# VITA-Group/SinNeRF

Measured on AMD Instinct MI355X. Metric: rendered rays/sec (64+64 samples), lego 400x400, higher is better.
Workload: dtype f32; 1 GPU; nerf_synthetic/lego-shaped 400x400 frame (160000 rays/GPU), N_samples=64, N_importance=64, eval render (perturb=0, noise_std=0, white_back), random-init teacher weights; points_per_ray=192, parallelism=rays sharded x1, no collective

## Files before the change

include/sinnerf_hip.h:

```cpp
#ifndef SINNERF_HIP_H
#define SINNERF_HIP_H
#include <stdint.h>
#ifdef __cplusplus
extern "C" {
#endif

#define SN_ABI_VERSION 5

#define SN_DTYPE_F32 0
#define SN_DTYPE_BF16 1
#define SN_DTYPE_BF16_STATE 2
#define SN_DTYPE_BF16X3 3
#define SN_DTYPE_F16 4
#define SN_DTYPE_CLASSIC_HEADS 0x100
#define SN_DTYPE_COMPILER_SCHEDULED 0x200
#define SN_DTYPE_EMB_BF16 0x400

#define SN_E_BADARG (-1)
#define SN_E_TOOLARGE (-2)
#define SN_E_MISSING_RNG (-3)
#define SN_E_UNSUPPORTED (-4)
#define SN_E_BADSHAPE (-5)

#define SN_FLAG_BF16_COMPILER_SCHEDULED 2
// ... 49 lines not shown
int sn_composite_backward(const float* raw, const float* z_vals, const float* rays, const float* noise, float noise_std,
                          long n_rays, int n_samples, int white_back, const float* g_rgb, const float* g_depth,
                          const float* g_weights, float* g_raw, void* stream);

long sn_ray_grads_workspace_bytes(long n_rays, int n_samples);
int sn_ray_grads(const float* w1, const float* w5, const float* wdir, int dtype, const void* g_acts, long slot_rows,
                 const float* rays, const float* z_vals, long n_rays, int n_samples, void* workspace, float* g_rays,
                 void* stream);

int sn_composite_backward_rays(const float* raw, const float* z_vals, const float* rays, const float* noise, float noise_std,
                               long n_rays, int n_samples, int white_back, const float* g_rgb, const float* g_depth,
                               const float* g_weights, float* g_raw, float* g_rays, void* stream);

int sn_mlp_forward_embedded(const void* blob, int dtype, const float* x, long n_rows, int ld, int sigma_only,
                            int flags, float* out, void* stream);

int sn_composite_forward(const float* raw, int has_rgb, const float* z_vals, const float* rays, const float* noise,
                         float noise_std, long n_rays, int n_samples, int white_back, float* rgb, float* depth,
                         float* weights, void* stream);

int sn_sample_pdf(const float* z_vals, const float* weights, const float* u, long n_rays, int n_samples,
                  int n_importance, float* z_fine, float* z_merged, void* stream);

int sn_sample_pdf_bins(const float* bins, const float* weights, const float* u, long n_rays, int n_bins,
                       int n_importance, float eps, float* samples, void* stream);


int sn_generate_rays(const float* c2w, int H, int W, float focal, float near, float far, int x0, int y0, int stride_x,
                     int stride_y, int patch_w, int patch_h, float* rays, void* stream);

long sn_generate_rays_backward_workspace_bytes(void);
int sn_generate_rays_backward(const float* g_rays, int H, int W, float focal, int x0, int y0, int stride_x, int stride_y,
                              int patch_w, int patch_h, void* workspace, float* g_c2w, void* stream);

int sn_adam_step(float* params, const float* grads, float* exp_avg, float* exp_avg_sq, long n, float lr, float beta1,
                 float beta2, float eps, float weight_decay, int step, void* stream);

long sn_render_loss_workspace_bytes(void);
int sn_render_loss(const float* rgb_coarse, const float* rgb_fine, const float* depth_coarse, const float* depth_fine,
                   const float* rgb_gt, const float* depth_gt, const unsigned char* mask, int mask_mode, long n,
                   float w_rgb, float w_depth, float* g_rgb_coarse, float* g_rgb_fine, float* g_depth_coarse,
                   float* g_depth_fine, void* workspace, float* out, void* stream);

#ifdef __cplusplus
}
#endif
// ... 2 lines not shown
```

sinnerf_amd/_lib.py:

```python
import ctypes
import os

_HERE = os.path.dirname(os.path.abspath(__file__))
LIB_PATH = os.environ.get("SINNERF_HIP_LIB") or os.path.join(_HERE, "csrc", "libsinnerf_hip.so")

SN_DTYPE_F32 = 0
SN_DTYPE_BF16 = 1
SN_DTYPE_BF16_STATE = 2
SN_DTYPE_BF16X3 = 3
SN_DTYPE_F16 = 4
SN_DTYPE_CLASSIC_HEADS = 0x100
SN_FLAG_F32_LDS_RING = 4
SN_DTYPE_COMPILER_SCHEDULED = 0x200
N_RAW_TENSORS = 24
SN_DTYPE_EMB_BF16 = 0x400
ABI_VERSION = 5

c_fp = ctypes.c_void_p
c_vp = ctypes.c_void_p
_long, _int, _float = ctypes.c_long, ctypes.c_int, ctypes.c_float

SIGNATURES = {
    "sn_abi_version": (_int, []),
    "sn_error_string": (ctypes.c_char_p, [_int]),
# ... 18 lines not shown
    "sn_sample_coarse": (_int, [c_fp, _long, _int, _int, _float, c_fp, c_fp, c_vp]),
    "sn_mlp_forward": (_int, [c_vp, _int, c_fp, c_fp, _long, _int, _int, _int, c_fp, c_vp]),
    "sn_mlp_forward_train": (_int, [c_vp, _int, c_fp, c_fp, _long, _int, c_fp, c_fp, c_fp, _long, c_vp]),
    "sn_mlp_forward_train_embedded": (_int, [c_vp, _int, c_fp, _long, _int, c_fp, c_fp, _long, c_vp]),
    "sn_mlp_backward_chain": (_int, [c_vp, _int, c_fp, c_fp, c_fp, _long, _long, c_fp, c_fp, c_vp]),
    "sn_dw_gemm": (_int, [c_vp, _int, c_vp]),
    "sn_weight_grads_workspace_bytes": (_long, [_long, _int]),
    "sn_weight_grads_plan": (_int, [_long, _int, c_vp, _int]),
    "sn_weight_grads": (_int, [c_vp, c_fp, c_vp, _long, _int, c_vp, ctypes.POINTER(c_vp), _int, c_vp]),
    "sn_generate_rays": (_int, [c_fp, _int, _int, _float, _float, _float, _int, _int, _int, _int, _int, _int, c_fp, c_vp]),
    "sn_adam_step": (_int, [c_fp, c_fp, c_fp, c_fp, _long, _float, _float, _float, _float, _float, _int, c_vp]),
    "sn_render_loss_workspace_bytes": (_long, []),
    "sn_render_loss": (_int, [c_fp, c_fp, c_fp, c_fp, c_fp, c_fp, c_vp, _int, _long, _float, _float, c_fp, c_fp, c_fp, c_fp,
                              c_vp, c_fp, c_vp]),
    "sn_composite_backward": (_int, [c_fp, c_fp, c_fp, c_fp, _float, _long, _int, _int, c_fp, c_fp, c_fp, c_fp, c_vp]),
    "sn_ray_grads_workspace_bytes": (_long, [_long, _int]),
    "sn_ray_grads": (_int, [c_fp, c_fp, c_fp, _int, c_vp, _long, c_fp, c_fp, _long, _int, c_vp, c_fp, c_vp]),
    "sn_composite_backward_rays": (_int, [c_fp, c_fp, c_fp, c_fp, _float, _long, _int, _int, c_fp, c_fp, c_fp, c_fp, c_fp, c_vp]),
    "sn_generate_rays_backward_workspace_bytes": (_long, []),
    "sn_generate_rays_backward": (_int, [c_fp, _int, _int, _float, _int, _int, _int, _int, _int, _int, c_vp, c_fp, c_vp]),
    "sn_mlp_forward_embedded": (_int, [c_vp, _int, c_fp, _long, _int, _int, _int, c_fp, c_vp]),
    "sn_composite_forward": (_int, [c_fp, _int, c_fp, c_fp, c_fp, _float, _long, _int, _int, c_fp, c_fp, c_fp, c_vp]),
    "sn_sample_pdf": (_int, [c_fp, c_fp, c_fp, _long, _int, _int, c_fp, c_fp, c_vp]),
    "sn_sample_pdf_bins": (_int, [c_fp, c_fp, c_fp, _long, _int, _int, _float, c_fp, c_vp]),
}


class SinnerfHipError(RuntimeError):
    pass


def _load():
    if not os.path.exists(LIB_PATH):
        raise ImportError(
            f"{LIB_PATH} not found: the HIP extension is not built. Run `python -c 'import __graft_entry__ as g; "
            "g.build()'` (or `make -C sinnerf_amd/csrc`). There is no CPU fallback for this path.")
    lib = ctypes.CDLL(LIB_PATH)
    for name, (res, args) in SIGNATURES.items():
        fn = getattr(lib, name)
        fn.restype, fn.argtypes = res, args
    if lib.sn_abi_version() != ABI_VERSION:
        raise ImportError(f"{LIB_PATH}: ABI version {lib.sn_abi_version()} != {ABI_VERSION}; rebuild the extension")
    return lib


lib = _load()
# ... 19 lines not shown
```

sinnerf_amd/csrc/sn_api.hip:

```cpp
#include <hip/hip_fp16.h>
#include "../../include/sinnerf_hip.h"
#include "sn_device.h"
#include "sn_layout.h"

extern "C" {
int sn_mlp_forward_f32_launch(const void* blob, const float* in0, const float* in1, long n_points, int s_or_ld,
                              int sigma_only, int input_mode, float* out, float* acts, float* emb,
                              long slot_rows, hipStream_t stream);
int sn_mlp_forward_f32g_launch(const void* blob, const float* in0, const float* in1, long n_points, int s_or_ld, int sigma_only,
                               int input_mode, float* out, float* acts, float* emb, long slot_rows, hipStream_t stream);
int sn_mlp_forward_f32g_classic_launch(const void* blob, const float* in0, const float* in1, long n_points, int s_or_ld, int sigma_only,
                                       int input_mode, float* out, float* acts, float* emb, long slot_rows, hipStream_t stream);
int sn_mlp_forward_f32g_store_launch(const void* blob, const float* in0, const float* in1, long n_points, int s_or_ld, int sigma_only,
                                     int input_mode, float* out, float* acts, float* emb, long slot_rows, hipStream_t stream);
int sn_mlp_forward_f32g_store_classic_launch(const void* blob, const float* in0, const float* in1, long n_points, int s_or_ld, int sigma_only,
                                             int input_mode, float* out, float* acts, float* emb, long slot_rows, hipStream_t stream);
int sn_mlp_forward_f32_classic_launch(const void* blob, const float* in0, const float* in1, long n_points, int s_or_ld,
                              int sigma_only, int input_mode, float* out, float* acts, float* emb,
                              long slot_rows, hipStream_t stream);
int sn_mlp_backward_chain_f32_launch(const void* bblob, const float* acts, const float* out_raw, const float* g_raw,
                                     long n_points, long slot_rows, float* G, float* g_out, hipStream_t stream);
int sn_mlp_backward_chain_f32_classic_launch(const void* bblob, const float* acts, const float* out_raw, const float* g_raw,
                                     long n_points, long slot_rows, float* G, float* g_out, hipStream_t stream);
int sn_mlp_backward_chain_f32g_launch(const void* bblob, const float* acts, const float* out_raw, const float* g_raw, long n_points,
// ... 67 lines not shown
                                                long n_points, long slot_rows, float* G, float* g_out, hipStream_t stream);
int sn_composite_backward_launch(const float* raw, const float* z_vals, const float* rays, const float* noise,
                                 float noise_std, long n_rays, int n_samples, int white_back, const float* g_rgb,
                                 const float* g_depth, const float* g_w, float* g_raw, hipStream_t stream);
int sn_composite_backward_rays_launch(const float* raw, const float* z_vals, const float* rays, const float* noise,
                                      float noise_std, long n_rays, int n_samples, int white_back, const float* g_rgb,
                                      const float* g_depth, const float* g_w, float* g_raw, float* g_rays, hipStream_t stream);
long sn_ray_grads_workspace_bytes_impl(long n_rays, int n_samples);
int sn_ray_grads_launch(const float* w1, const float* w5, const float* wdir, int layout, const void* g_acts, long slot_rows,
                        const float* rays, const float* z_vals, long n_rays, int n_samples, void* workspace, float* g_rays,
                        hipStream_t stream);
long sn_generate_rays_backward_workspace_bytes_impl();
int sn_generate_rays_backward_launch(const float* g_rays, int H, int W, float focal, int x0, int y0, int sx, int sy, int pw,
                                     int ph, void* workspace, float* g_c2w, hipStream_t stream);
int sn_sample_coarse_launch(const float* rays, long n_rays, int n_samples, int use_disp, float perturb,
                            const float* perturb_rand, float* z_out, hipStream_t stream);
int sn_composite_forward_launch(const float* raw, int has_rgb, const float* z_vals, const float* rays,
                                const float* noise, float noise_std, long n_rays, int n_samples, int white_back,
                                float* rgb, float* depth, float* weights, hipStream_t stream);
int sn_sample_pdf_launch(const float* z_vals, const float* weights, const float* u, long n_rays, int n_samples,
                         int n_importance, float* z_fine, float* z_merged, hipStream_t stream);
int sn_sample_pdf_bins_launch(const float* bins, const float* weights, const float* u, long n_rays, int n_bins,
                              int n_importance, float eps, float* samples, hipStream_t stream);
}

namespace {
struct RawPtrs { const float* p[snl::N_RAW]; };

__device__ __forceinline__ unsigned short f32_to_bf16_rne(float f) {
  unsigned int u = __float_as_uint(f);
  if ((u & 0x7fffffffu) > 0x7f800000u) return (unsigned short)((u >> 16) | 0x40);
  u += 0x7fffu + ((u >> 16) & 1u);
  return (unsigned short)(u >> 16);
}

__global__ void __launch_bounds__(256)
pack_kernel(RawPtrs raw, const snl::PackEntry* __restrict__ table, long n, char* __restrict__ blob, int dtype) {
  for (long i = (long)blockIdx.x * blockDim.x + threadIdx.x; i < n; i += (long)gridDim.x * blockDim.x) {
    const snl::PackEntry e = table[i];
    float v = 0.0f;
    const bool as_f32 = (e.src == -2) || (e.src >= 0 && (e.src & snl::SRC_F32_FLAG));
    if (e.src >= 0) {
      const int t = (e.src >> 20) & 0x1ff, off = e.src & 0xfffff;
      const float* src = raw.p[0];
#pragma unroll
      for (int k = 1; k < snl::N_RAW; ++k) src = (t == k) ? raw.p[k] : src;
// ... 323 lines not shown
    return SN_HEADS(classic, sn_mlp_forward_bf16)(blob, x, nullptr, n_rows, ld, sigma_only, 1, out, nullptr, nullptr, 0, 0, (hipStream_t)stream);
  if (dtype != SN_DTYPE_F32) return SN_E_UNSUPPORTED;
  if (!(flags & SN_FLAG_F32_LDS_RING))
    return SN_HEADS(classic, sn_mlp_forward_f32g)(blob, x, nullptr, n_rows, ld, sigma_only, 1, out, nullptr, nullptr, 0, (hipStream_t)stream);
  return SN_HEADS(classic, sn_mlp_forward_f32)(blob, x, nullptr, n_rows, ld, sigma_only, 1,
                                               out, nullptr, nullptr, 0, (hipStream_t)stream);
}

int sn_composite_forward(const float* raw, int has_rgb, const float* z_vals, const float* rays, const float* noise,
                         float noise_std, long n_rays, int n_samples, int white_back, float* rgb, float* depth,
                         float* weights, void* stream) {
  if (!raw || !z_vals || !rays || !weights || n_rays < 0 || n_samples < 1) return SN_E_BADARG;
  if (has_rgb && (!rgb || !depth)) return SN_E_BADARG;
  return sn_composite_forward_launch(raw, has_rgb, z_vals, rays, noise, noise_std, n_rays, n_samples, white_back, rgb,
                                     depth, weights, (hipStream_t)stream);
}

int sn_sample_pdf(const float* z_vals, const float* weights, const float* u, long n_rays, int n_samples,
                  int n_importance, float* z_fine, float* z_merged, void* stream) {
  if (!z_vals || !weights || !z_merged || n_rays < 0) return SN_E_BADARG;
  return sn_sample_pdf_launch(z_vals, weights, u, n_rays, n_samples, n_importance, z_fine, z_merged, (hipStream_t)stream);
}

int sn_sample_pdf_bins(const float* bins, const float* weights, const float* u, long n_rays, int n_bins,
                       int n_importance, float eps, float* samples, void* stream) {
  if (!bins || !weights || !samples || n_rays < 0 || !(eps > 0.0f)) return SN_E_BADARG;
  return sn_sample_pdf_bins_launch(bins, weights, u, n_rays, n_bins, n_importance, eps, samples, (hipStream_t)stream);
}

}
```

sinnerf_amd/csrc/sn_render.hip:

```cpp
#include "sn_device.h"

namespace snr {

SN_DEV float linspace01(int i, int n) {
  if (n <= 1) return 0.0f;
  const float step = __fdiv_rn(1.0f, (float)(n - 1));
  return (i < n / 2) ? __fmul_rn((float)i, step) : __builtin_fmaf(-(float)(n - 1 - i), step, 1.0f);
}

SN_DEV float coarse_z(float near, float far, float t, int use_disp) {
  const float omt = __fsub_rn(1.0f, t);
  if (!use_disp) return __fadd_rn(__fmul_rn(near, omt), __fmul_rn(far, t));
  const float a = __fmul_rn(__fdiv_rn(1.0f, near), omt), b = __fmul_rn(__fdiv_rn(1.0f, far), t);
  return __fdiv_rn(1.0f, __fadd_rn(a, b));
}

__global__ void __launch_bounds__(256)
sample_coarse_kernel(const float* __restrict__ rays, long n_rays, int S, int use_disp, float perturb,
                     const float* __restrict__ perturb_rand, float* __restrict__ z_out) {
  const long total = n_rays * (long)S;
  for (long idx = (long)blockIdx.x * blockDim.x + threadIdx.x; idx < total; idx += (long)gridDim.x * blockDim.x) {
    const long ray = idx / S;
    const int i = (int)(idx - ray * S);
    const float near = rays[ray * 8 + 6], far = rays[ray * 8 + 7];
// ... 19 lines not shown
  return v;
}
SN_DEV double wave_incl_scan_add(double v, int lane) {
#pragma unroll
  for (int off = 1; off < 64; off <<= 1) {
    const double o = __shfl_up(v, off, 64);
    if (lane >= off) v += o;
  }
  return v;
}
SN_DEV double wave_sum(double v) {
#pragma unroll
  for (int off = 32; off > 0; off >>= 1) v += __shfl_xor(v, off, 64);
  return v;
}

SN_DEV void wave_lds_sync() {
  __builtin_amdgcn_fence(__ATOMIC_RELEASE, "wavefront");
  __builtin_amdgcn_wave_barrier();
  __builtin_amdgcn_fence(__ATOMIC_ACQUIRE, "wavefront");
}

template <int C, bool HAS_RGB>
__global__ void __launch_bounds__(256)
composite_fwd_kernel(const float* __restrict__ raw, const float* __restrict__ z_vals, const float* __restrict__ rays,
                     const float* __restrict__ noise, float noise_std, long n_rays, int S, int white_back,
                     float* __restrict__ rgb_out, float* __restrict__ depth_out, float* __restrict__ w_out) {
  const int lane = threadIdx.x & 63;
  const long ray = (long)blockIdx.x * 4 + (threadIdx.x >> 6);
  if (ray >= n_rays) return;
  const float dx = rays[ray * 8 + 3], dy = rays[ray * 8 + 4], dz = rays[ray * 8 + 5];
  const float dnorm = __fsqrt_rn(__fadd_rn(__fadd_rn(__fmul_rn(dx, dx), __fmul_rn(dy, dy)), __fmul_rn(dz, dz)));
  const long base = ray * (long)S;
  const int i0 = lane * C;

  float z[C + 1], sg[C], cr[C], cg[C], cb[C];
#pragma unroll
  for (int c = 0; c < C + 1; ++c) {
    const int i = i0 + c;
    z[c] = (i < S) ? z_vals[base + i] : 0.0f;
  }
#pragma unroll
  for (int c = 0; c < C; ++c) {
    const int i = i0 + c;
    if (i < S) {
      if (HAS_RGB) {
        const float4 v = reinterpret_cast<const float4*>(raw)[base + i];
        cr[c] = v.x; cg[c] = v.y; cb[c] = v.z; sg[c] = v.w;
      } else {
        sg[c] = raw[base + i];
        cr[c] = cg[c] = cb[c] = 0.0f;
      }
    } else {
      sg[c] = cr[c] = cg[c] = cb[c] = 0.0f;
    }
  }
  float alpha[C];
  double fprod = 1.0;
#pragma unroll
  for (int c = 0; c < C; ++c) {
    const int i = i0 + c;
    float a = 0.0f, f = 1.0f;
    if (i < S) {
      float delta = (i < S - 1) ? __fsub_rn(z[c + 1], z[c]) : 1e10f;
      delta = __fmul_rn(delta, dnorm);
      float s = sg[c];
      if (noise != nullptr) s = __fadd_rn(s, __fmul_rn(noise[base + i], noise_std));
      s = fmaxf(s, 0.0f);
      a = __fsub_rn(1.0f, expf(__fmul_rn(-delta, s)));
      f = __fadd_rn(__fsub_rn(1.0f, a), 1e-10f);
    }
    alpha[c] = a;
    fprod *= (double)f;
  }
  const double incl = wave_incl_scan_mul(fprod, lane);
  double t = __shfl_up(incl, 1, 64);
  if (lane == 0) t = 1.0;
  double wsum = 0.0, sr = 0.0, sgc = 0.0, sb = 0.0, sd = 0.0;
#pragma unroll
  for (int c = 0; c < C; ++c) {
    const int i = i0 + c;
    const float w = __fmul_rn(alpha[c], (float)t);
    if (i < S) {
      w_out[base + i] = w;
      wsum += (double)w;
      if (HAS_RGB) {
        sr += (double)__fmul_rn(w, cr[c]);
        sgc += (double)__fmul_rn(w, cg[c]);
        sb += (double)__fmul_rn(w, cb[c]);
        sd += (double)__fmul_rn(w, z[c]);
      }
      const float a = alpha[c];
      t *= (double)__fadd_rn(__fsub_rn(1.0f, a), 1e-10f);
    }
  }
  if (HAS_RGB) {
    wsum = wave_sum(wsum); sr = wave_sum(sr); sgc = wave_sum(sgc); sb = wave_sum(sb); sd = wave_sum(sd);
    if (lane == 0) {
      float r = (float)sr, g = (float)sgc, b = (float)sb;
      if (white_back) {
        const float ws = (float)wsum;
        r = __fsub_rn(__fadd_rn(r, 1.0f), ws);
        g = __fsub_rn(__fadd_rn(g, 1.0f), ws);
        b = __fsub_rn(__fadd_rn(b, 1.0f), ws);
      }
      rgb_out[ray * 3 + 0] = r; rgb_out[ray * 3 + 1] = g; rgb_out[ray * 3 + 2] = b;
      depth_out[ray] = (float)sd;
    }
  }
}

template <int C, bool RAYS>
SN_DEV void composite_bwd_body(const float* __restrict__ raw, const float* __restrict__ z_vals, const float* __restrict__ rays,
                               const float* __restrict__ noise, float noise_std, long n_rays, int S, int white_back,
                               const float* __restrict__ g_rgb, const float* __restrict__ g_depth,
                               const float* __restrict__ g_w, float* __restrict__ g_raw, float* __restrict__ g_rays) {
  const int lane = threadIdx.x & 63;
  const long ray = (long)blockIdx.x * 4 + (threadIdx.x >> 6);
  if (ray >= n_rays) return;
  const float dx = rays[ray * 8 + 3], dy = rays[ray * 8 + 4], dz = rays[ray * 8 + 5];
  const float dnorm = __fsqrt_rn(__fadd_rn(__fadd_rn(__fmul_rn(dx, dx), __fmul_rn(dy, dy)), __fmul_rn(dz, dz)));
  const long base = ray * (long)S;
  const int i0 = lane * C;
  const float gr = g_rgb ? g_rgb[ray * 3 + 0] : 0.0f, gg = g_rgb ? g_rgb[ray * 3 + 1] : 0.0f,
              gb = g_rgb ? g_rgb[ray * 3 + 2] : 0.0f, gd = g_depth ? g_depth[ray] : 0.0f;
  const float gwhite = white_back ? (gr + gg + gb) : 0.0f;

  float zc[C + 1];
#pragma unroll
  for (int c = 0; c < C + 1; ++c) zc[c] = (i0 + c < S) ? z_vals[base + i0 + c] : 0.0f;
  float alpha[C], ex[C], dl[C], Gi[C], fi[C];
  float dzs[C], sps[C];
// ... 62 lines not shown
      reinterpret_cast<float4*>(g_rays)[ray * 2] = lo;
      reinterpret_cast<float4*>(g_rays)[ray * 2 + 1] = hi;
    }
  }
}

template <int C>
__global__ void __launch_bounds__(256)
composite_bwd_kernel(const float* __restrict__ raw, const float* __restrict__ z_vals, const float* __restrict__ rays,
                     const float* __restrict__ noise, float noise_std, long n_rays, int S, int white_back,
                     const float* __restrict__ g_rgb, const float* __restrict__ g_depth, const float* __restrict__ g_w,
                     float* __restrict__ g_raw) {
  composite_bwd_body<C, false>(raw, z_vals, rays, noise, noise_std, n_rays, S, white_back, g_rgb, g_depth, g_w, g_raw, nullptr);
}
template <int C>
__global__ void __launch_bounds__(256)
composite_bwd_rays_kernel(const float* __restrict__ raw, const float* __restrict__ z_vals, const float* __restrict__ rays,
                          const float* __restrict__ noise, float noise_std, long n_rays, int S, int white_back,
                          const float* __restrict__ g_rgb, const float* __restrict__ g_depth, const float* __restrict__ g_w,
                          float* __restrict__ g_raw, float* __restrict__ g_rays) {
  composite_bwd_body<C, true>(raw, z_vals, rays, noise, noise_std, n_rays, S, white_back, g_rgb, g_depth, g_w, g_raw, g_rays);
}

template <bool FROM_Z>
__global__ void __launch_bounds__(256)
sample_pdf_kernel(const float* __restrict__ z_vals, const float* __restrict__ weights, const float* __restrict__ u_in,
                  long n_rays, int S, int NI, float eps, float* __restrict__ z_fine_out, float* __restrict__ z_merged_out) {
  extern __shared__ __attribute__((aligned(16))) char smem[];
  const int lane = threadIdx.x & 63;
  const int wv = threadIdx.x >> 6;
  const long ray = (long)blockIdx.x * 4 + wv;
  const int M = S - 2;
  const int L = S - 1;
  const int n = S + NI;
  const int per_wave = 2 * L + n + (FROM_Z ? n : 0);
  float* cdf = reinterpret_cast<float*>(smem) + (long)wv * per_wave;
  float* bins = cdf + L;
  float* keys = bins + L;
  float* merged = keys + n;
  if (ray >= n_rays) return;
  const long base = FROM_Z ? ray * (long)S : ray * (long)M - 1;

  const int C = (M + 63) / 64;
  double local = 0.0;
  for (int c = 0; c < C; ++c) {
    const int k = lane * C + c;
    if (k < M) local += (double)__fadd_rn(weights[base + k + 1], eps);
  }
  const float tot = (float)wave_sum(local);
  double run = 0.0;
  for (int c = 0; c < C; ++c) {
    const int k = lane * C + c;
    if (k < M) run += (double)__fdiv_rn(__fadd_rn(weights[base + k + 1], eps), tot);
  }
  const double incl = wave_incl_scan_add(run, lane);
  double acc = incl - run;
  for (int c = 0; c < C; ++c) {
    const int k = lane * C + c;
    if (k < M) {
      acc += (double)__fdiv_rn(__fadd_rn(weights[base + k + 1], eps), tot);
      cdf[k + 1] = (float)acc;
    }
  }
  if (lane == 0) cdf[0] = 0.0f;
  if (FROM_Z) {
    for (int k = lane; k < L; k += 64)
      bins[k] = __fmul_rn(0.5f, __fadd_rn(z_vals[base + k], z_vals[base + k + 1]));
    for (int k = lane; k < S; k += 64) keys[k] = z_vals[base + k];
  } else {
    for (int k = lane; k < L; k += 64) bins[k] = z_vals[ray * (long)L + k];
  }
  wave_lds_sync();

  for (int i = lane; i < NI; i += 64) {
    const float u = (u_in != nullptr) ? u_in[ray * (long)NI + i] : linspace01(i, NI);
    int lo = 0, hi = L;
    while (lo < hi) {
      const int mid = (lo + hi) >> 1;
      if (cdf[mid] <= u) lo = mid + 1; else hi = mid;
    }
    const int inds = lo;
    const int below = max(inds - 1, 0);
    const int above = min(inds, M);
    const float c0 = cdf[below], c1 = cdf[above], b0 = bins[below], b1 = bins[above];
    float denom = __fsub_rn(c1, c0);
    if (denom < eps) denom = 1.0f;
    const float smp = __fadd_rn(b0, __fmul_rn(__fdiv_rn(__fsub_rn(u, c0), denom), __fsub_rn(b1, b0)));
    keys[S + i] = smp;
    if (z_fine_out != nullptr) z_fine_out[ray * (long)NI + i] = smp;
  }
  if (!FROM_Z) return;
  wave_lds_sync();
  bool ascending = true;
  for (int i = lane; i < NI - 1; i += 64) ascending = ascending && (keys[S + i] <= keys[S + i + 1]);
  for (int i = lane; i < S - 1; i += 64) ascending = ascending && (keys[i] <= keys[i + 1]);
  if (__all(ascending)) {
    const float* kf = keys + S;
    for (int i = lane; i < S; i += 64) {
      const float k = keys[i];
      int lo = 0, hi = NI;
      while (lo < hi) {
        const int mid = (lo + hi) >> 1;
        if (kf[mid] < k) lo = mid + 1; else hi = mid;
      }
      merged[i + lo] = k;
    }
    for (int m = lane; m < NI; m += 64) {
      const float k = kf[m];
      int lo = 0, hi = S;
      while (lo < hi) {
        const int mid = (lo + hi) >> 1;
        if (keys[mid] <= k) lo = mid + 1; else hi = mid;
      }
      merged[m + lo] = k;
    }
  } else {
    for (int i = lane; i < n; i += 64) {
      const float k = keys[i];
      int rank = 0;
      for (int j = 0; j < n; ++j) {
        const float kj = keys[j];
        rank += (kj < k || (kj == k && j < i)) ? 1 : 0;
      }
      merged[rank] = k;
    }
  }
  wave_lds_sync();
  for (int i = lane; i < n; i += 64) z_merged_out[ray * (long)n + i] = merged[i];
}

}

extern "C" int sn_sample_coarse_launch(const float* rays, long n_rays, int n_samples, int use_disp, float perturb,
                                       const float* perturb_rand, float* z_out, hipStream_t stream) {
  if (n_rays <= 0) return 0;
  if (perturb > 0.0f && perturb_rand == nullptr) return -3;
  const long total = n_rays * (long)n_samples;
  long blocks = (total + 255) / 256;
  if (blocks > 256 * 16) blocks = 256 * 16;
  hipLaunchKernelGGL(snr::sample_coarse_kernel, dim3((unsigned)blocks), dim3(256), 0, stream, rays, n_rays, n_samples,
                     use_disp, perturb, perturb_rand, z_out);
  return (int)hipGetLastError();
}

extern "C" int sn_composite_forward_launch(const float* raw, int has_rgb, const float* z_vals, const float* rays,
                                           const float* noise, float noise_std, long n_rays, int n_samples,
                                           int white_back, float* rgb, float* depth, float* weights,
                                           hipStream_t stream) {
  using namespace snr;
  if (n_rays <= 0) return 0;
  const int C = (n_samples + 63) / 64;
// ... 52 lines not shown
    hipLaunchKernelGGL((composite_bwd_rays_kernel<CC>), grid, block, 0, stream, raw, z_vals, rays, noise, noise_std, n_rays, \
                       n_samples, white_back, g_rgb, g_depth, g_w, g_raw, g_rays);                               \
    break;
  switch (C) { SN_CBR(1) SN_CBR(2) SN_CBR(3) SN_CBR(4) SN_CBR(5) SN_CBR(6) SN_CBR(7) SN_CBR(8) SN_CBR(9) SN_CBR(10) SN_CBR(11)
               SN_CBR(12) SN_CBR(13) SN_CBR(14) SN_CBR(15) SN_CBR(16) }
#undef SN_CBR
  return (int)hipGetLastError();
}

extern "C" int sn_sample_pdf_launch(const float* z_vals, const float* weights, const float* u, long n_rays,
                                    int n_samples, int n_importance, float* z_fine, float* z_merged,
                                    hipStream_t stream) {
  if (n_rays <= 0) return 0;
  if (n_samples < 3 || n_importance < 1) return -5;
  const long blocks = (n_rays + 3) / 4;
  if (blocks > 0x7fffffffL) return -2;
  const size_t lds = 4 * (size_t)(2 * (n_samples - 1) + 2 * (n_samples + n_importance)) * sizeof(float);
  if (lds > 64 * 1024) return -4;
  hipLaunchKernelGGL(snr::sample_pdf_kernel<true>, dim3((unsigned)blocks), dim3(256), lds, stream, z_vals, weights, u,
                     n_rays, n_samples, n_importance, 1e-5f , z_fine, z_merged);
  return (int)hipGetLastError();
}

extern "C" int sn_sample_pdf_bins_launch(const float* bins, const float* weights, const float* u, long n_rays,
                                         int n_bins, int n_importance, float eps, float* samples, hipStream_t stream) {
  if (n_rays <= 0) return 0;
  if (n_bins < 1 || n_importance < 1) return -5;
  const int S = n_bins + 2;
  const long blocks = (n_rays + 3) / 4;
  if (blocks > 0x7fffffffL) return -2;
  const size_t lds = 4 * (size_t)(2 * (S - 1) + S + n_importance) * sizeof(float);
  if (lds > 64 * 1024) return -4;
  hipLaunchKernelGGL(snr::sample_pdf_kernel<false>, dim3((unsigned)blocks), dim3(256), lds, stream, bins, weights, u,
                     n_rays, S, n_importance, eps, samples, (float*)nullptr);
  return (int)hipGetLastError();
}
```

sinnerf_amd/rendering.py:

```python
import torch

from . import _lib
from .nerf import NeRF, dtype_code

__all__ = ["render_rays", "sample_pdf"]

PROFILE = None


MAX_FUSED_SAMPLES = 1024


def _is_pow2_bands(e, in_channels, n_freqs):
    fb = getattr(e, "freq_bands", None)
    if isinstance(fb, torch.Tensor):
        key = (id(fb), fb._version, fb.data_ptr(), tuple(fb.shape), str(fb.device), in_channels, n_freqs)
        if fb.device.type == "cpu" and fb.numel() <= 16:
            key += (tuple(fb.detach().reshape(-1).tolist()),)
    else:
        try:
            key = (tuple(float(v) for v in fb), in_channels, n_freqs) if fb is not None else (None, in_channels, n_freqs)
        except TypeError:
            key = (id(fb), in_channels, n_freqs)
    hit = getattr(e, "_sn_pow2_verdict", None)
    if hit is not None and hit[0] == key:
        return hit[1]
    ok = (fb is not None and getattr(e, "in_channels", None) == in_channels and getattr(e, "N_freqs", None) == n_freqs
          and len(fb) == n_freqs)
    if ok:
        host = torch.as_tensor(fb).detach().to("cpu", torch.float64)
        ok = bool(torch.equal(host, 2.0 ** torch.arange(n_freqs, dtype=torch.float64)))
# ... 57 lines not shown
        res.update(rgb_coarse=e(0, 3), depth_coarse=e(0))
    elif N_importance == 0:
        raise NameError("name 'rgb_coarse' is not defined (rendering.py:331)")
    res.update(rgb_fine=e(0, 3), depth_fine=e(0), opacity_fine=e(0, sf))
    return res


def _forward_core(models, rays, N_samples, use_disp, perturb, noise_std, N_importance, white_back, test_time,
                  flags=0, keep=None):
    dev = rays.device
    n = rays.shape[0]
    if n == 0:
        return _empty_result(dev, N_samples, N_importance, test_time)
    stream = _lib.stream_ptr()
    perturb_rand = None
    if perturb > 0:
        perturb_rand = torch.rand((n, N_samples), device=dev)
    z_vals = torch.empty((n, N_samples), dtype=torch.float32, device=dev)
    _lib.check(_lib.lib.sn_sample_coarse(_lib.ptr(rays), n, N_samples, int(bool(use_disp)), float(perturb),
                                         _lib.ptr(perturb_rand), _lib.ptr(z_vals), stream), "sn_sample_coarse")
    result = {}
    raw_c = _mlp(models[0], rays, z_vals, sigma_only=bool(test_time), flags=flags)
    noise_c = torch.randn((n, N_samples), device=dev)
    rgb_c, depth_c, w_c = _composite(raw_c, not test_time, z_vals, rays, noise_c if noise_std != 0 else None,
                                     noise_std, white_back)
    if test_time:
        result["opacity_coarse"] = w_c
    else:
        result.update(rgb_coarse=rgb_c, depth_coarse=depth_c, opacity_coarse=w_c)
    if keep is not None:
        keep.update(z_coarse=z_vals, raw_coarse=raw_c, noise_coarse=noise_c if noise_std != 0 else None)
    if N_importance > 0:
        u = torch.rand((n, N_importance), device=dev) if perturb > 0 else None
        z_all = torch.empty((n, N_samples + N_importance), dtype=torch.float32, device=dev)
        _lib.check(_lib.lib.sn_sample_pdf(_lib.ptr(z_vals), _lib.ptr(w_c), _lib.ptr(u), n, N_samples, N_importance,
                                          None, _lib.ptr(z_all), stream), "sn_sample_pdf")
        raw_f = _mlp(models[1], rays, z_all, sigma_only=False, flags=flags)
        noise_f = torch.randn((n, N_samples + N_importance), device=dev)
        rgb_f, depth_f, w_f = _composite(raw_f, True, z_all, rays, noise_f if noise_std != 0 else None, noise_std,
                                         white_back)
        result.update(rgb_fine=rgb_f, depth_fine=depth_f, opacity_fine=w_f)
        if keep is not None:
            keep.update(z_fine=z_all, raw_fine=raw_f, noise_fine=noise_f if noise_std != 0 else None)
    else:
        if test_time:
            raise NameError("name 'rgb_coarse' is not defined (render_rays(test_time=True) needs N_importance > 0, "
                            "as in the reference: rendering.py:331)")
        result.update(rgb_fine=rgb_c, depth_fine=depth_c, opacity_fine=w_c)
    return result


def render_rays(models,
                embeddings,
                rays,
                N_samples=64,
                use_disp=False,
                perturb=0,
                noise_std=1,
                N_importance=0,
# ... 59 lines not shown
```

Before: 661,600 rays/s.

## Fuse coarse compositing with PDF importance sampling into one persistent kernel

```diff
diff --git a/include/sinnerf_hip.h b/include/sinnerf_hip.h
--- a/include/sinnerf_hip.h
+++ b/include/sinnerf_hip.h
@@ -95,6 +95,10 @@
 int sn_sample_pdf(const float* z_vals, const float* weights, const float* u, long n_rays, int n_samples,
                   int n_importance, float* z_fine, float* z_merged, void* stream);
 
+int sn_coarse_tail(const float* raw, int has_rgb, const float* z_vals, const float* rays, const float* noise, float noise_std,
+                   const float* u, long n_rays, int n_samples, int n_importance, int white_back, float* rgb, float* depth,
+                   float* weights, float* z_all, void* stream);
+
 int sn_sample_pdf_bins(const float* bins, const float* weights, const float* u, long n_rays, int n_bins,
                        int n_importance, float eps, float* samples, void* stream);
 
diff --git a/sinnerf_amd/_lib.py b/sinnerf_amd/_lib.py
--- a/sinnerf_amd/_lib.py
+++ b/sinnerf_amd/_lib.py
@@ -64,6 +64,7 @@
     "sn_mlp_forward_embedded": (_int, [c_vp, _int, c_fp, _long, _int, _int, _int, c_fp, c_vp]),
     "sn_composite_forward": (_int, [c_fp, _int, c_fp, c_fp, c_fp, _float, _long, _int, _int, c_fp, c_fp, c_fp, c_vp]),
     "sn_sample_pdf": (_int, [c_fp, c_fp, c_fp, _long, _int, _int, c_fp, c_fp, c_vp]),
+    "sn_coarse_tail": (_int, [c_fp, _int, c_fp, c_fp, c_fp, _float, c_fp, _long, _int, _int, _int, c_fp, c_fp, c_fp, c_fp, c_vp]),
     "sn_sample_pdf_bins": (_int, [c_fp, c_fp, c_fp, _long, _int, _int, _float, c_fp, c_vp]),
 }
 
diff --git a/sinnerf_amd/csrc/sn_api.hip b/sinnerf_amd/csrc/sn_api.hip
--- a/sinnerf_amd/csrc/sn_api.hip
+++ b/sinnerf_amd/csrc/sn_api.hip
@@ -113,6 +113,9 @@
                          int n_importance, float* z_fine, float* z_merged, hipStream_t stream);
 int sn_sample_pdf_bins_launch(const float* bins, const float* weights, const float* u, long n_rays, int n_bins,
                               int n_importance, float eps, float* samples, hipStream_t stream);
+int sn_coarse_tail_launch(const float* raw, int has_rgb, const float* z_vals, const float* rays, const float* noise,
+                          float noise_std, const float* u, long n_rays, int n_samples, int n_importance, int white_back,
+                          float* rgb, float* depth, float* weights, float* z_all, hipStream_t stream);
 }
 
 namespace {
@@ -482,6 +485,15 @@
   return sn_sample_pdf_launch(z_vals, weights, u, n_rays, n_samples, n_importance, z_fine, z_merged, (hipStream_t)stream);
 }
 
+int sn_coarse_tail(const float* raw, int has_rgb, const float* z_vals, const float* rays, const float* noise, float noise_std,
+                   const float* u, long n_rays, int n_samples, int n_importance, int white_back, float* rgb, float* depth,
+                   float* weights, float* z_all, void* stream) {
+  if (!raw || !z_vals || !rays || !weights || !z_all || n_rays < 0 || n_samples < 1) return SN_E_BADARG;
+  if (has_rgb && (!rgb || !depth)) return SN_E_BADARG;
+  return sn_coarse_tail_launch(raw, has_rgb, z_vals, rays, noise, noise_std, u, n_rays, n_samples, n_importance, white_back,
+                               rgb, depth, weights, z_all, (hipStream_t)stream);
+}
+
 int sn_sample_pdf_bins(const float* bins, const float* weights, const float* u, long n_rays, int n_bins,
                        int n_importance, float eps, float* samples, void* stream) {
   if (!bins || !weights || !samples || n_rays < 0 || !(eps > 0.0f)) return SN_E_BADARG;
diff --git a/sinnerf_amd/csrc/sn_render.hip b/sinnerf_amd/csrc/sn_render.hip
--- a/sinnerf_amd/csrc/sn_render.hip
+++ b/sinnerf_amd/csrc/sn_render.hip
@@ -1,4 +1,5 @@
 #include "sn_device.h"
+#include "sn_launch.h"
 
 namespace snr {
 
@@ -65,39 +66,40 @@
 }
 
 template <int C, bool HAS_RGB>
-__global__ void __launch_bounds__(256)
-composite_fwd_kernel(const float* __restrict__ raw, const float* __restrict__ z_vals, const float* __restrict__ rays,
-                     const float* __restrict__ noise, float noise_std, long n_rays, int S, int white_back,
-                     float* __restrict__ rgb_out, float* __restrict__ depth_out, float* __restrict__ w_out) {
-  const int lane = threadIdx.x & 63;
-  const long ray = (long)blockIdx.x * 4 + (threadIdx.x >> 6);
-  if (ray >= n_rays) return;
-  const float dx = rays[ray * 8 + 3], dy = rays[ray * 8 + 4], dz = rays[ray * 8 + 5];
-  const float dnorm = __fsqrt_rn(__fadd_rn(__fadd_rn(__fmul_rn(dx, dx), __fmul_rn(dy, dy)), __fmul_rn(dz, dz)));
+struct CompIn {
+  float z[C + 1], sg[C], nz[C];
+  float cr[HAS_RGB ? C : 1], cg[HAS_RGB ? C : 1], cb[HAS_RGB ? C : 1];
+  float dx, dy, dz;
+};
+
+template <int C, bool HAS_RGB>
+SN_DEV void comp_load(CompIn<C, HAS_RGB>& in, const float* __restrict__ raw, const float* __restrict__ z_vals,
+                      const float* __restrict__ rays, const float* __restrict__ noise, long ray, int S, int lane) {
+  in.dx = rays[ray * 8 + 3]; in.dy = rays[ray * 8 + 4]; in.dz = rays[ray * 8 + 5];
   const long base = ray * (long)S;
   const int i0 = lane * C;
-
-  float z[C + 1], sg[C], cr[C], cg[C], cb[C];
-#pragma unroll
-  for (int c = 0; c < C + 1; ++c) {
-    const int i = i0 + c;
-    z[c] = (i < S) ? z_vals[base + i] : 0.0f;
-  }
+#pragma unroll
+  for (int c = 0; c < C + 1; ++c) in.z[c] = z_vals[base + min(i0 + c, S - 1)];
 #pragma unroll
   for (int c = 0; c < C; ++c) {
-    const int i = i0 + c;
-    if (i < S) {
-      if (HAS_RGB) {
-        const float4 v = reinterpret_cast<const float4*>(raw)[base + i];
-        cr[c] = v.x; cg[c] = v.y; cb[c] = v.z; sg[c] = v.w;
-      } else {
-        sg[c] = raw[base + i];
-        cr[c] = cg[c] = cb[c] = 0.0f;
-      }
+    const long at = base + min(i0 + c, S - 1);
+    if (HAS_RGB) {
+      const float4 v = reinterpret_cast<const float4*>(raw)[at];
+      in.cr[c] = v.x; in.cg[c] = v.y; in.cb[c] = v.z; in.sg[c] = v.w;
     } else {
-      sg[c] = cr[c] = cg[c] = cb[c] = 0.0f;
-    }
-  }
+      in.sg[c] = raw[at];
+    }
+    in.nz[c] = 0.0f;
+    if (noise != nullptr) in.nz[c] = noise[at];
+  }
+}
+
+template <int C, bool HAS_RGB>
+SN_DEV void comp_body(const CompIn<C, HAS_RGB>& in, bool has_noise, float noise_std, long ray, int S, int lane, int white_back,
+                      float (&w)[C], float* __restrict__ rgb_out, float* __restrict__ depth_out) {
+  const float dx = in.dx, dy = in.dy, dz = in.dz;
+  const float dnorm = __fsqrt_rn(__fadd_rn(__fadd_rn(__fmul_rn(dx, dx), __fmul_rn(dy, dy)), __fmul_rn(dz, dz)));
+  const int i0 = lane * C;
   float alpha[C];
   double fprod = 1.0;
 #pragma unroll
@@ -105,10 +107,10 @@
     const int i = i0 + c;
     float a = 0.0f, f = 1.0f;
     if (i < S) {
-      float delta = (i < S - 1) ? __fsub_rn(z[c + 1], z[c]) : 1e10f;
+      float delta = (i < S - 1) ? __fsub_rn(in.z[c + 1], in.z[c]) : 1e10f;
       delta = __fmul_rn(delta, dnorm);
-      float s = sg[c];
-      if (noise != nullptr) s = __fadd_rn(s, __fmul_rn(noise[base + i], noise_std));
+      float s = in.sg[c];
+      if (has_noise) s = __fadd_rn(s, __fmul_rn(in.nz[c], noise_std));
       s = fmaxf(s, 0.0f);
       a = __fsub_rn(1.0f, expf(__fmul_rn(-delta, s)));
       f = __fadd_rn(__fsub_rn(1.0f, a), 1e-10f);
@@ -123,15 +125,14 @@
 #pragma unroll
   for (int c = 0; c < C; ++c) {
     const int i = i0 + c;
-    const float w = __fmul_rn(alpha[c], (float)t);
+    w[c] = __fmul_rn(alpha[c], (float)t);
     if (i < S) {
-      w_out[base + i] = w;
-      wsum += (double)w;
       if (HAS_RGB) {
-        sr += (double)__fmul_rn(w, cr[c]);
-        sgc += (double)__fmul_rn(w, cg[c]);
-        sb += (double)__fmul_rn(w, cb[c]);
-        sd += (double)__fmul_rn(w, z[c]);
+        wsum += (double)w[c];
+        sr += (double)__fmul_rn(w[c], in.cr[c]);
+        sgc += (double)__fmul_rn(w[c], in.cg[c]);
+        sb += (double)__fmul_rn(w[c], in.cb[c]);
+        sd += (double)__fmul_rn(w[c], in.z[c]);
       }
       const float a = alpha[c];
       t *= (double)__fadd_rn(__fsub_rn(1.0f, a), 1e-10f);
@@ -151,6 +152,24 @@
       depth_out[ray] = (float)sd;
     }
   }
+}
+
+template <int C, bool HAS_RGB>
+__global__ void __launch_bounds__(256)
+composite_fwd_kernel(const float* __restrict__ raw, const float* __restrict__ z_vals, const float* __restrict__ rays,
+                     const float* __restrict__ noise, float noise_std, long n_rays, int S, int white_back,
+                     float* __restrict__ rgb_out, float* __restrict__ depth_out, float* __restrict__ w_out) {
+  const int lane = threadIdx.x & 63;
+  const long ray = (long)blockIdx.x * 4 + (threadIdx.x >> 6);
+  if (ray >= n_rays) return;
+  CompIn<C, HAS_RGB> in;
+  comp_load<C, HAS_RGB>(in, raw, z_vals, rays, noise, ray, S, lane);
+  float w[C];
+  comp_body<C, HAS_RGB>(in, noise != nullptr, noise_std, ray, S, lane, white_back, w, rgb_out, depth_out);
+  const long base = ray * (long)S;
+#pragma unroll
+  for (int c = 0; c < C; ++c)
+    if (lane * C + c < S) w_out[base + lane * C + c] = w[c];
 }
 
 template <int C, bool RAYS>
@@ -259,6 +278,115 @@
   composite_bwd_body<C, true>(raw, z_vals, rays, noise, noise_std, n_rays, S, white_back, g_rgb, g_depth, g_w, g_raw, g_rays);
 }
 
+SN_DEV float z_mid(float a, float b) { return __fmul_rn(0.5f, __fadd_rn(a, b)); }
+
+SN_DEV void pdf_to_cdf(const float* pw, int M, float eps, int lane, float* cdf) {
+  const int CB = (M + 63) / 64;
+  double local = 0.0;
+#pragma unroll 1
+  for (int c = 0; c < CB; ++c) {
+    const int k = lane * CB + c;
+    if (k < M) local += (double)__fadd_rn(pw[k], eps);
+  }
+  const float tot = (float)wave_sum(local);
+  double run = 0.0;
+#pragma unroll 1
+  for (int c = 0; c < CB; ++c) {
+    const int k = lane * CB + c;
+    if (k < M) run += (double)__fdiv_rn(__fadd_rn(pw[k], eps), tot);
+  }
+  const double incl = wave_incl_scan_add(run, lane);
+  double acc = incl - run;
+#pragma unroll 1
+  for (int c = 0; c < CB; ++c) {
+    const int k = lane * CB + c;
+    if (k < M) {
+      acc += (double)__fdiv_rn(__fadd_rn(pw[k], eps), tot);
+      cdf[k + 1] = (float)acc;
+    }
+  }
+  if (lane == 0) cdf[0] = 0.0f;
+}
+
+SN_DEV float pdf_sample(const float* cdf, const float* bins, int L, int M, float eps, float u) {
+  int lo = 0, hi = L;
+  while (lo < hi) {
+    const int mid = (lo + hi) >> 1;
+    if (cdf[mid] <= u) lo = mid + 1; else hi = mid;
+  }
+  const int inds = lo;
+  const int below = max(inds - 1, 0);
+  const int above = min(inds, M);
+  const float c0 = cdf[below], c1 = cdf[above], b0 = bins[below], b1 = bins[above];
+  float denom = __fsub_rn(c1, c0);
+  if (denom < eps) denom = 1.0f;
+  return __fadd_rn(b0, __fmul_rn(__fdiv_rn(__fsub_rn(u, c0), denom), __fsub_rn(b1, b0)));
+}
+
+template <int UPRE>
+SN_DEV void pdf_search(const float* cdf, const float* bins, const float* __restrict__ urow, const float (&upre)[UPRE > 0 ? UPRE : 1],
+                       int NI, int L, int M, float eps, int lane, float* samples, float* __restrict__ z_fine_row) {
+#pragma unroll
+  for (int j = 0; j < UPRE; ++j) {
+    const int i = lane + 64 * j;
+    if (i < NI) {
+      const float smp = pdf_sample(cdf, bins, L, M, eps, (urow != nullptr) ? upre[j] : linspace01(i, NI));
+      samples[i] = smp;
+      if (z_fine_row != nullptr) z_fine_row[i] = smp;
+    }
+  }
+#pragma unroll 1
+  for (int i = lane + 64 * UPRE; i < NI; i += 64) {
+    const float smp = pdf_sample(cdf, bins, L, M, eps, (urow != nullptr) ? urow[i] : linspace01(i, NI));
+    samples[i] = smp;
+    if (z_fine_row != nullptr) z_fine_row[i] = smp;
+  }
+}
+
+SN_DEV void merge_by_rank(const float* keys, float* merged, int S, int NI, int lane) {
+  const int n = S + NI;
+  bool ascending = true;
+#pragma unroll 1
+  for (int i = lane; i < NI - 1; i += 64) ascending = ascending && (keys[S + i] <= keys[S + i + 1]);
+#pragma unroll 1
+  for (int i = lane; i < S - 1; i += 64) ascending = ascending && (keys[i] <= keys[i + 1]);
+  if (__all(ascending)) {
+    const float* kf = keys + S;
+#pragma unroll 1
+    for (int i = lane; i < S; i += 64) {
+      const float k = keys[i];
+      int lo = 0, hi = NI;
+      while (lo < hi) {
+        const int mid = (lo + hi) >> 1;
+        if (kf[mid] < k) lo = mid + 1; else hi = mid;
+      }
+      merged[i + lo] = k;
+    }
+#pragma unroll 1
+    for (int m = lane; m < NI; m += 64) {
+      const float k = kf[m];
+      int lo = 0, hi = S;
+      while (lo < hi) {
+        const int mid = (lo + hi) >> 1;
+        if (keys[mid] <= k) lo = mid + 1; else hi = mid;
+      }
+      merged[m + lo] = k;
+    }
+  } else {
+#pragma unroll 1
+    for (int i = lane; i < n; i += 64) {
+      const float k = keys[i];
+      int rank = 0;
+#pragma unroll 1
+      for (int j = 0; j < n; ++j) {
+        const float kj = keys[j];
+        rank += (kj < k || (kj == k && j < i)) ? 1 : 0;
+      }
+      merged[rank] = k;
+    }
+  }
+}
+
 template <bool FROM_Z>
 __global__ void __launch_bounds__(256)
 sample_pdf_kernel(const float* __restrict__ z_vals, const float* __restrict__ weights, const float* __restrict__ u_in,
@@ -278,92 +406,118 @@
   if (ray >= n_rays) return;
   const long base = FROM_Z ? ray * (long)S : ray * (long)M - 1;
 
-  const int C = (M + 63) / 64;
-  double local = 0.0;
-  for (int c = 0; c < C; ++c) {
-    const int k = lane * C + c;
-    if (k < M) local += (double)__fadd_rn(weights[base + k + 1], eps);
-  }
-  const float tot = (float)wave_sum(local);
-  double run = 0.0;
-  for (int c = 0; c < C; ++c) {
-    const int k = lane * C + c;
-    if (k < M) run += (double)__fdiv_rn(__fadd_rn(weights[base + k + 1], eps), tot);
-  }
-  const double incl = wave_incl_scan_add(run, lane);
-  double acc = incl - run;
-  for (int c = 0; c < C; ++c) {
-    const int k = lane * C + c;
-    if (k < M) {
-      acc += (double)__fdiv_rn(__fadd_rn(weights[base + k + 1], eps), tot);
-      cdf[k + 1] = (float)acc;
-    }
-  }
-  if (lane == 0) cdf[0] = 0.0f;
+  pdf_to_cdf(weights + (base + 1), M, eps, lane, cdf);
   if (FROM_Z) {
-    for (int k = lane; k < L; k += 64)
-      bins[k] = __fmul_rn(0.5f, __fadd_rn(z_vals[base + k], z_vals[base + k + 1]));
+    for (int k = lane; k < L; k += 64) bins[k] = z_mid(z_vals[base + k], z_vals[base + k + 1]);
     for (int k = lane; k < S; k += 64) keys[k] = z_vals[base + k];
   } else {
     for (int k = lane; k < L; k += 64) bins[k] = z_vals[ray * (long)L + k];
   }
   wave_lds_sync();
-
-  for (int i = lane; i < NI; i += 64) {
-    const float u = (u_in != nullptr) ? u_in[ray * (long)NI + i] : linspace01(i, NI);
-    int lo = 0, hi = L;
-    while (lo < hi) {
-      const int mid = (lo + hi) >> 1;
-      if (cdf[mid] <= u) lo = mid + 1; else hi = mid;
-    }
-    const int inds = lo;
-    const int below = max(inds - 1, 0);
-    const int above = min(inds, M);
-    const float c0 = cdf[below], c1 = cdf[above], b0 = bins[below], b1 = bins[above];
-    float denom = __fsub_rn(c1, c0);
-    if (denom < eps) denom = 1.0f;
-    const float smp = __fadd_rn(b0, __fmul_rn(__fdiv_rn(__fsub_rn(u, c0), denom), __fsub_rn(b1, b0)));
-    keys[S + i] = smp;
-    if (z_fine_out != nullptr) z_fine_out[ray * (long)NI + i] = smp;
-  }
+  const float no_u[1] = {0.0f};
+  pdf_search<0>(cdf, bins, (u_in != nullptr) ? u_in + ray * (long)NI : nullptr, no_u, NI, L, M, eps, lane, keys + S,
+                (z_fine_out != nullptr) ? z_fine_out + ray * (long)NI : nullptr);
   if (!FROM_Z) return;
   wave_lds_sync();
-  bool ascending = true;
-  for (int i = lane; i < NI - 1; i += 64) ascending = ascending && (keys[S + i] <= keys[S + i + 1]);
-  for (int i = lane; i < S - 1; i += 64) ascending = ascending && (keys[i] <= keys[i + 1]);
-  if (__all(ascending)) {
-    const float* kf = keys + S;
-    for (int i = lane; i < S; i += 64) {
-      const float k = keys[i];
-      int lo = 0, hi = NI;
-      while (lo < hi) {
-        const int mid = (lo + hi) >> 1;
-        if (kf[mid] < k) lo = mid + 1; else hi = mid;
-      }
-      merged[i + lo] = k;
-    }
-    for (int m = lane; m < NI; m += 64) {
-      const float k = kf[m];
-      int lo = 0, hi = S;
-      while (lo < hi) {
-        const int mid = (lo + hi) >> 1;
-        if (keys[mid] <= k) lo = mid + 1; else hi = mid;
-      }
-      merged[m + lo] = k;
-    }
-  } else {
-    for (int i = lane; i < n; i += 64) {
-      const float k = keys[i];
-      int rank = 0;
-      for (int j = 0; j < n; ++j) {
-        const float kj = keys[j];
-        rank += (kj < k || (kj == k && j < i)) ? 1 : 0;
-      }
-      merged[rank] = k;
-    }
-  }
+  merge_by_rank(keys, merged, S, NI, lane);
   wave_lds_sync();
   for (int i = lane; i < n; i += 64) z_merged_out[ray * (long)n + i] = merged[i];
+}
+
+#ifndef SN_TAIL_WAVES_LE2
+#define SN_TAIL_WAVES_LE2 8
+#endif
+#define TAIL_WAVES(C) ((C) <= 2 ? SN_TAIL_WAVES_LE2 : (C) <= 4 ? 4 : 1)
+constexpr int TAIL_UPRE = 2;
+
+template <int C, bool HAS_RGB>
+__global__ void __launch_bounds__(256, TAIL_WAVES(C))
+coarse_tail_kernel(const float* __restrict__ raw, const float* __restrict__ z_vals, const float* __restrict__ rays,
+                   const float* __restrict__ noise, float noise_std, const float* __restrict__ u_in, long n_rays, int S, int NI,
+                   int white_back, float eps, float* __restrict__ rgb_out, float* __restrict__ depth_out,
+                   float* __restrict__ w_out, float* __restrict__ z_all_out) {
+  extern __shared__ __attribute__((aligned(16))) char smem[];
+  constexpr bool PREFETCH = (C <= 2);
+  const int lane = threadIdx.x & 63;
+  const int wv = __builtin_amdgcn_readfirstlane(threadIdx.x >> 6);
+  const int M = S - 2, L = S - 1, n = S + NI;
+  const int per_wave = 2 * L + 2 * n;
+  float* cdf = reinterpret_cast<float*>(smem) + (long)wv * per_wave;
+  float* bins = cdf + L;
+  float* keys = bins + L;
+  float* merged = keys + n;
+  float* wl = merged;
+  const long stride = (long)gridDim.x * 4;
+  long ray = (long)blockIdx.x * 4 + wv;
+  if (ray >= n_rays) return;
+
+  auto load_u = [&](float (&uu)[TAIL_UPRE], long r, int lane) __attribute__((always_inline)) {
+#pragma unroll
+    for (int j = 0; j < TAIL_UPRE; ++j) {
+      uu[j] = 0.0f;
+      if (u_in != nullptr) uu[j] = u_in[r * (long)NI + min(lane + 64 * j, NI - 1)];
+    }
+  };
+  auto settle = [&](CompIn<C, HAS_RGB>& in, float (&uu)[TAIL_UPRE]) __attribute__((always_inline)) {
+#pragma unroll
+    for (int c = 0; c < C + 1; ++c) asm volatile("" : "+v"(in.z[c]));
+#pragma unroll
+    for (int c = 0; c < C; ++c) {
+      asm volatile("" : "+v"(in.sg[c]), "+v"(in.nz[c]));
+      if (HAS_RGB) asm volatile("" : "+v"(in.cr[c]), "+v"(in.cg[c]), "+v"(in.cb[c]));
+    }
+    asm volatile("" : "+v"(in.dx), "+v"(in.dy), "+v"(in.dz));
+#pragma unroll
+    for (int j = 0; j < TAIL_UPRE; ++j) asm volatile("" : "+v"(uu[j]));
+  };
+  CompIn<C, HAS_RGB> cur, nxt;
+  float ucur[TAIL_UPRE], unxt[TAIL_UPRE];
+  comp_load<C, HAS_RGB>(cur, raw, z_vals, rays, noise, ray, S, lane);
+  load_u(ucur, ray, lane);
+  __builtin_amdgcn_s_waitcnt(0x0f70);
+  const int lane0 = lane;
+  while (true) {
+    int lane = lane0;
+    asm volatile("" : "+v"(lane));
+    const long next = ray + stride;
+    const bool more = next < n_rays;
+    if (PREFETCH && more) {
+      comp_load<C, HAS_RGB>(nxt, raw, z_vals, rays, noise, next, S, lane);
+      load_u(unxt, next, lane);
+    }
+    float w[C];
+    comp_body<C, HAS_RGB>(cur, noise != nullptr, noise_std, ray, S, lane, white_back, w, rgb_out, depth_out);
+#pragma unroll
+    for (int c = 0; c < C; ++c) {
+      const int i = lane * C + c;
+      if (i < S) {
+        wl[i] = w[c];
+        keys[i] = cur.z[c];
+        if (i < L) bins[i] = z_mid(cur.z[c], cur.z[c + 1]);
+      }
+    }
+    wave_lds_sync();
+    for (int i = lane; i < S; i += 64) w_out[ray * (long)S + i] = wl[i];
+    pdf_to_cdf(wl + 1, M, eps, lane, cdf);
+    wave_lds_sync();
+    pdf_search<TAIL_UPRE>(cdf, bins, (u_in != nullptr) ? u_in + ray * (long)NI : nullptr, ucur, NI, L, M, eps, lane, keys + S,
+                          nullptr);
+    wave_lds_sync();
+    merge_by_rank(keys, merged, S, NI, lane);
+    wave_lds_sync();
+    if (PREFETCH && more) settle(nxt, unxt);
+    for (int i = lane; i < n; i += 64) z_all_out[ray * (long)n + i] = merged[i];
+    if (!more) break;
+    wave_lds_sync();
+    ray = next;
+    if (PREFETCH) {
+      cur = nxt;
+      for (int j = 0; j < TAIL_UPRE; ++j) ucur[j] = unxt[j];
+    } else {
+      comp_load<C, HAS_RGB>(cur, raw, z_vals, rays, noise, ray, S, lane);
+      load_u(ucur, ray, lane);
+    }
+  }
 }
 
 }
@@ -462,6 +616,53 @@
   return (int)hipGetLastError();
 }
 
+namespace snr {
+template <int C, bool HAS_RGB>
+int coarse_tail_launch(const float* raw, const float* z_vals, const float* rays, const float* noise, float noise_std,
+                       const float* u, long n_rays, int S, int NI, int white_back, float* rgb, float* depth, float* weights,
+                       float* z_all, size_t lds, hipStream_t stream) {
+  static int by_regs[snh::MAX_DEVICES];
+  const int dev = snh::current_device();
+  int per_cu = dev >= 0 ? __atomic_load_n(&by_regs[dev], __ATOMIC_RELAXED) : 0;
+  if (per_cu == 0) {
+    if (hipOccupancyMaxActiveBlocksPerMultiprocessor(&per_cu, coarse_tail_kernel<C, HAS_RGB>, 256, 0) != hipSuccess || per_cu < 1)
+      per_cu = 1;
+    if (per_cu > TAIL_WAVES(C)) per_cu = TAIL_WAVES(C);
+    if (dev >= 0) __atomic_store_n(&by_regs[dev], per_cu, __ATOMIC_RELAXED);
+  }
+  const long by_lds = (long)(160 * 1024 / lds);
+  long blocks = (n_rays + 3) / 4;
+  const long resident = (long)snh::cu_count() * (per_cu < by_lds ? per_cu : by_lds);
+  if (blocks > resident) blocks = resident;
+  hipLaunchKernelGGL((coarse_tail_kernel<C, HAS_RGB>), dim3((unsigned)blocks), dim3(256), lds, stream, raw, z_vals, rays, noise,
+                     noise_std, u, n_rays, S, NI, white_back, 1e-5f , rgb, depth, weights, z_all);
+  return (int)hipGetLastError();
+}
+}
+
+extern "C" int sn_coarse_tail_launch(const float* raw, int has_rgb, const float* z_vals, const float* rays, const float* noise,
+                                     float noise_std, const float* u, long n_rays, int n_samples, int n_importance,
+                                     int white_back, float* rgb, float* depth, float* weights, float* z_all,
+                                     hipStream_t stream) {
+  using namespace snr;
+  if (n_rays <= 0) return 0;
+  if (n_samples < 3 || n_importance < 1) return -5;
+  const int C = (n_samples + 63) / 64;
+  if (C > 16 || (long)n_samples + n_importance > 1024) return -4;
+  const size_t lds = 4 * (size_t)(2 * (n_samples - 1) + 2 * (n_samples + n_importance)) * sizeof(float);
+  if (lds > 64 * 1024) return -4;
+#define SN_CT(CC)                                                                                                \
+  case CC:                                                                                                       \
+    return has_rgb ? coarse_tail_launch<CC, true>(raw, z_vals, rays, noise, noise_std, u, n_rays, n_samples, n_importance,     \
+                                                  white_back, rgb, depth, weights, z_all, lds, stream)           \
+                   : coarse_tail_launch<CC, false>(raw, z_vals, rays, noise, noise_std, u, n_rays, n_samples, n_importance,    \
+                                                   white_back, rgb, depth, weights, z_all, lds, stream);
+  switch (C) { SN_CT(1) SN_CT(2) SN_CT(3) SN_CT(4) SN_CT(5) SN_CT(6) SN_CT(7) SN_CT(8) SN_CT(9) SN_CT(10) SN_CT(11) SN_CT(12)
+               SN_CT(13) SN_CT(14) SN_CT(15) SN_CT(16) }
+#undef SN_CT
+  return -4;
+}
+
 extern "C" int sn_sample_pdf_bins_launch(const float* bins, const float* weights, const float* u, long n_rays,
                                          int n_bins, int n_importance, float eps, float* samples, hipStream_t stream) {
   if (n_rays <= 0) return 0;
diff --git a/sinnerf_amd/rendering.py b/sinnerf_amd/rendering.py
--- a/sinnerf_amd/rendering.py
+++ b/sinnerf_amd/rendering.py
@@ -7,6 +7,8 @@
 
 PROFILE = None
 
+
+FUSED_COARSE_TAIL = True
 
 MAX_FUSED_SAMPLES = 1024
 
@@ -110,8 +112,21 @@
     result = {}
     raw_c = _mlp(models[0], rays, z_vals, sigma_only=bool(test_time), flags=flags)
     noise_c = torch.randn((n, N_samples), device=dev)
-    rgb_c, depth_c, w_c = _composite(raw_c, not test_time, z_vals, rays, noise_c if noise_std != 0 else None,
-                                     noise_std, white_back)
+    fused = N_importance > 0 and (FUSED_COARSE_TAIL == "always" or (FUSED_COARSE_TAIL is True and not perturb > 0))
+    if fused:
+        u = torch.rand((n, N_importance), device=dev) if perturb > 0 else None
+        has_rgb = not test_time
+        w_c = torch.empty((n, N_samples), dtype=torch.float32, device=dev)
+        rgb_c = torch.empty((n, 3), dtype=torch.float32, device=dev) if has_rgb else None
+        depth_c = torch.empty((n,), dtype=torch.float32, device=dev) if has_rgb else None
+        z_all = torch.empty((n, N_samples + N_importance), dtype=torch.float32, device=dev)
+        _lib.check(_lib.lib.sn_coarse_tail(_lib.ptr(raw_c), int(has_rgb), _lib.ptr(z_vals), _lib.ptr(rays),
+                                           _lib.ptr(noise_c if noise_std != 0 else None), float(noise_std), _lib.ptr(u), n,
+                                           N_samples, N_importance, int(bool(white_back)), _lib.ptr(rgb_c), _lib.ptr(depth_c),
+                                           _lib.ptr(w_c), _lib.ptr(z_all), stream), "sn_coarse_tail")
+    else:
+        rgb_c, depth_c, w_c = _composite(raw_c, not test_time, z_vals, rays, noise_c if noise_std != 0 else None,
+                                         noise_std, white_back)
     if test_time:
         result["opacity_coarse"] = w_c
     else:
@@ -119,10 +134,11 @@
     if keep is not None:
         keep.update(z_coarse=z_vals, raw_coarse=raw_c, noise_coarse=noise_c if noise_std != 0 else None)
     if N_importance > 0:
-        u = torch.rand((n, N_importance), device=dev) if perturb > 0 else None
-        z_all = torch.empty((n, N_samples + N_importance), dtype=torch.float32, device=dev)
-        _lib.check(_lib.lib.sn_sample_pdf(_lib.ptr(z_vals), _lib.ptr(w_c), _lib.ptr(u), n, N_samples, N_importance,
-                                          None, _lib.ptr(z_all), stream), "sn_sample_pdf")
+        if not fused:
+            u = torch.rand((n, N_importance), device=dev) if perturb > 0 else None
+            z_all = torch.empty((n, N_samples + N_importance), dtype=torch.float32, device=dev)
+            _lib.check(_lib.lib.sn_sample_pdf(_lib.ptr(z_vals), _lib.ptr(w_c), _lib.ptr(u), n, N_samples, N_importance,
+                                              None, _lib.ptr(z_all), stream), "sn_sample_pdf")
         raw_f = _mlp(models[1], rays, z_all, sigma_only=False, flags=flags)
         noise_f = torch.randn((n, N_samples + N_importance), device=dev)
         rgb_f, depth_f, w_f = _composite(raw_f, True, z_all, rays, noise_f if noise_std != 0 else None, noise_std,
```

New measurement: 661,700 rays/s, median of 2. Within noise of the previous version (+0.0%).
